# alexmillerdb/two_tower_recommender_model

Hardware: AMD Instinct MI355X
Metric: training pairs/sec at batch 8192 (per GPU) (higher is better)
Workload: dtype fp32; 1 GPU; northstar: 100M items x 50M users, emb_dim 128, towers [128, 64], single-hot uniform ids; global_batch=8192, per_gpu_batch=8192, emb_dim=128, tower_dtype=bf16 (MFMA, fp32 acc), parallelism=single-gpu hipgraph

## Files before the change

two_tower_recommender_model_amd/csrc/tower.hip:

```cpp
#include <vector>

#include "tt_common.h"
#include "dedup.h"
#include "shard.h"

namespace tt {

typedef __attribute__((ext_vector_type(8))) __bf16 bf16x8;
typedef __attribute__((ext_vector_type(4))) float f32x4;
typedef __attribute__((ext_vector_type(4))) __bf16 bf16x4;

constexpr int TR = 32;
constexpr int MAXW = 128;
constexpr int XCH = 128;
constexpr int LSTR = MAXW + 8;
constexpr int FSTR = MAXW + 4;
constexpr int MAXL = 4;

__device__ __forceinline__ int64_t strip_at(int64_t f, int64_t m, int64_t nf) {
  return (((m >> 5) * nf + f) << 5) + (m & 31);
}

struct TowerArgs {
  tt_tower_shape_t s;
  int64_t B;
  const float* pooled;
  int64_t ldp;
  float* gpooled;
  const float* params;
  const __bf16* wb;
  const __bf16* wtb;
  const __bf16* wbf;
  const __bf16* wtbf;
  int64_t woff[2][MAXL];
  int64_t boff[2][MAXL];
  int64_t wcoff[2][MAXL];
  const void* labels;
  int label_dtype;
  float grad_scale;
  float* logits;
  __bf16* xt;
  __bf16* act;
  __bf16* dzt;
  float* dbpart;
  float* loss_part;
  int64_t in_max;
  int64_t Bp;
  int nwg;
  const void* gcol[2];
  const float* gtab[2];
  int64_t gmod[2];
  int gid_dtype;
  float* pooled_out;
  DedupWs dd;
  int dd_on;
  int dd_table[2];
  const int32_t* gpos[2];
  const float* gsrc[2];
  float* gdst[2];
  const int32_t* gpos_out[2];
  int gsrc_bf16;
  float* uw[2];
  float* us[2];
  float ulr, ueps;
  const void* pcol[2];
  const void* mval;
  const int32_t* moff[2];
  const int32_t* ipos;
  const int32_t* ipos_out;
  const __bf16* isrc;
  float* idst;
  int ifeat0[2];
  int iD;
  const char* wimg;
  tt_peer_direct_t xd;
#if TT_EXPERIMENTS
// ... 1063 lines not shown
  for (int q = 1; q < TT_PEER_MAXW; ++q) {
    if (q < x.W && row >= x.first_row[q]) {
      base = reinterpret_cast<char*>(x.row0[q]);
      f0 = x.first_row[q];
    }
  }
  return base + (row - f0) * row_bytes;
}
__device__ __forceinline__ bool px_copy_unit(const tt_peer_direct_t& x, int64_t u, const uint4*& src, uint4*& dst) {
  int64_t pre = 0;
  bool hit = false;
#pragma unroll
  for (int q = 0; q < TT_PEER_MAXW; ++q) {
    const int64_t n = q < x.W ? x.copy_len[q] >> 4 : 0;
    if (!hit && u >= pre && u < pre + n) {
      src = reinterpret_cast<const uint4*>(x.copy_src[q]) + (u - pre);
      dst = reinterpret_cast<uint4*>(x.copy_dst[q]) + (u - pre);
      hit = true;
    }
    pre += n;
  }
  return hit;
}
__device__ __forceinline__ int64_t px_copy_units(const tt_peer_direct_t& x) {
  int64_t n = 0;
#pragma unroll
  for (int q = 0; q < TT_PEER_MAXW; ++q) n += q < x.W ? x.copy_len[q] >> 4 : 0;
  return n;
}

struct RkRaw {
  uint32_t lo, hi;
};
__device__ __forceinline__ RkRaw rk_raw(const void* p, bool wide, int64_t i) {
  RkRaw r;
  if (wide) {
    const uint2 v = reinterpret_cast<const uint2*>(p)[i];
    r.lo = v.x;
    r.hi = v.y;
  } else {
    r.lo = reinterpret_cast<const uint32_t*>(p)[i];
    r.hi = 0u;
  }
  return r;
}
__device__ __forceinline__ int64_t rk_id(RkRaw r, bool wide) {
  return wide ? (int64_t)(((uint64_t)r.hi << 32) | r.lo) : (int64_t)(int32_t)r.lo;
}
__device__ __forceinline__ float rk_label(RkRaw r, int dt) {
  if (dt == TT_I32) return (float)(int32_t)r.lo;
  if (dt == TT_I64) return (float)(int64_t)(((uint64_t)r.hi << 32) | r.lo);
  return __uint_as_float(r.lo);
}
#if TT_EXPERIMENTS
#define RK_STAMP(k) \
  do { if (a.stamps && lane == 0) a.stamps[8192 + ((int64_t)blockIdx.x * 16 + (k)) * 9 + wid] = (int64_t)__builtin_amdgcn_s_memrealtime(); } while (0)
#define RK_STAMP2(k) \
  do { if (a.stamps && lane == 0) a.stamps[8192 + ((int64_t)blockIdx.x * 16 + (k)) * 9 + 4 + wid] = (int64_t)__builtin_amdgcn_s_memrealtime(); } while (0)
#define RK_STAMP_IMG(k) \
  do { if (a.stamps && lane == 0) a.stamps[8192 + ((int64_t)blockIdx.x * 16 + (k)) * 9 + 8] = (int64_t)__builtin_amdgcn_s_memrealtime(); } while (0)
#else
#define RK_STAMP(k) do { } while (0)
#define RK_STAMP2(k) do { } while (0)
#define RK_STAMP_IMG(k) do { } while (0)
#endif

typedef uint32_t t3_u32x4 __attribute__((ext_vector_type(4)));
constexpr int T3_NSEG = 2 * 2 * MAXL;

struct alignas(64) UpdateArgs {
  float* params;
  float* exp_avg;
  float* exp_avg_sq;
  const float* slab;
  const float* adam_pre;
  const float* grads_in;
  int32_t P;
  int S;
  int do_adam;
  int nseg;
  t3_u32x4 seg[T3_NSEG];
  const float* dbpart;
  int nwg;
  __bf16* wb;
  __bf16* wtb;
  __bf16* wbf;
  __bf16* wtbf;
  int skip_plain;
  float lr, beta1, beta2, eps, wd;
  int64_t* step_state;
  float* grads_out;
  int out_copies;
  int64_t out_stride;
  int64_t out_off[16];
  float out_scale;
  int in_srcs;
  int64_t in_stride;
  char* wimg;
  PxWait wt;
#if TT_EXPERIMENTS
  int64_t* stamps;
#endif
};
#if TT_EXPERIMENTS
#define T3_BLOCK ((int)blockDim.x)
#else
// ... 58 lines not shown
    m = m + (1.f - a.beta1) * (g - m);
    const float v = v0 * a.beta2 + (1.f - a.beta2) * g * g;
    const float denom = sqrtf(v) / bc2_sqrt + a.eps;
    p = p + (-step_size) * m / denom;
    a.exp_avg[i] = m;
    a.exp_avg_sq[i] = v;
    a.params[i] = p;
  }
  if (sg.sisw) {
    const int K = sg.sk, N = sg.sn;
    const int64_t n = e / K, k = e - n * K;
    if (!a.skip_plain) {
      a.wb[sg.swc + e] = (__bf16)p;
      a.wtb[sg.swc + k * N + n] = (__bf16)p;
    }
    a.wbf[sg.swc + frag_off((int)n, (int)k, K)] = (__bf16)p;
    a.wtbf[sg.swc + frag_off((int)k, (int)n, N)] = (__bf16)p;
    if (a.wimg)
      *reinterpret_cast<__bf16*>(a.wimg + sg.st_ * RK_IMG_T + sg.sl_ * (RK_W0 * 256) + rk_off((int)n, (int)k)) = (__bf16)p;
  }
}

template <bool UPD, bool IDX, int IN, bool POOL = false>
__device__ __forceinline__ void tower_rows_body(const TowerArgs& a) {
  static_assert(IN == 128 || IN == 64, "row-owned T1: inputs of 128 or 64");
  static_assert(!POOL || (!UPD && !IDX), "pooled input: the plain T1 only");
  constexpr int NI = IN / 32;
  constexpr int MTI = IN / 16;
  __shared__ __attribute__((aligned(16))) char wimg[RK_IMG];
  __shared__ __attribute__((aligned(16))) float xo[2][2][16 * 64];
  __shared__ float bsum[2][RK_W0 + RK_W1];
  __shared__ float lrow[TR];
  __shared__ __attribute__((aligned(16))) float xr[4][16 * IN];
  const int lane = threadIdx.x & 63, wid = __builtin_amdgcn_readfirstlane(threadIdx.x >> 6);
  typedef __attribute__((address_space(3))) void lds_void;
  typedef __attribute__((address_space(1))) void glb_void;
  if (wid == 4) {
    RK_STAMP_IMG(0);
    if (!TDBG(16)) {
#pragma unroll
      for (int k = 0; k < RK_IMG / 1024; ++k)
        __builtin_amdgcn_global_load_lds((glb_void*)(a.wimg + k * 1024 + lane * 16), (lds_void*)(wimg + k * 1024), 16, 0, 0);
    }
    RK_STAMP_IMG(1);
    __builtin_amdgcn_s_waitcnt(0x0F70);
    RK_STAMP_IMG(2);
    __syncthreads();
    RK_STAMP_IMG(3);
    __syncthreads();
    __syncthreads();
    return;
  }
  const int t = wid >> 1, h = wid & 1, q = lane >> 4, n = lane & 15;
  const int tile = xcd_remap((int)blockIdx.x, (int)gridDim.x);
  const int64_t B = a.B, m0 = (int64_t)tile * TR, m = m0 + 16 * h + n;
  const bool live = m < B;
  RK_STAMP(0);
  const bool wide = a.gid_dtype == TT_I64;
  const int64_t mc = live ? m : 0;
  RkRaw id_raw{0u, 0u}, pout_raw{0u, 0u};
  if (IDX) {
    id_raw.lo = (uint32_t)(t ? a.gpos[1] : a.gpos[0])[mc];
    pout_raw.lo = a.gpos_out[0] ? (uint32_t)(t ? a.gpos_out[1] : a.gpos_out[0])[mc] : id_raw.lo;
  } else if (!POOL) {
    id_raw = rk_raw(t ? a.gcol[1] : a.gcol[0], wide, mc);
  }
  int32_t cl = -1;
  if (UPD) cl = a.dd.claim[live ? t * B + m : 0];
  const RkRaw lab_raw = rk_raw(a.labels, a.label_dtype == TT_I64, mc);
  f32x4 b0v[8], b1v[4];
  auto load_biases = [&]() {
    const float* b0p = a.params + a.boff[t][0];
    const float* b1p = a.params + a.boff[t][1];
#pragma unroll
    for (int mt = 0; mt < 8; ++mt) b0v[mt] = *reinterpret_cast<const f32x4*>(b0p + 32 * (mt >> 1) + 8 * q + 4 * (mt & 1));
#pragma unroll
    for (int mt = 0; mt < 4; ++mt) b1v[mt] = *reinterpret_cast<const f32x4*>(b1p + 32 * (mt >> 1) + 8 * q + 4 * (mt & 1));
  };
  load_biases();
  __builtin_amdgcn_sched_barrier(0);
  uint4 cpv = make_uint4(0u, 0u, 0u, 0u);
  uint4* cpd = nullptr;
  int64_t cp_per = 0, cp_end = 0;
  if constexpr (IDX) {
    if (a.xd.W) {
      const int64_t tot = px_copy_units(a.xd);
      cp_per = (tot + gridDim.x - 1) / gridDim.x;
      cp_end = min(tot, ((int64_t)blockIdx.x + 1) * cp_per);
      const int64_t u = (int64_t)blockIdx.x * cp_per + threadIdx.x;
      const uint4* cps;
      if (u < cp_end && px_copy_unit(a.xd, u, cps, cpd)) cpv = *cps;
      else cpd = nullptr;
    }
  }
  int64_t r;
  if (POOL) {
    r = live ? m : -1;
  } else if (IDX) {
    r = live ? (int64_t)(int32_t)id_raw.lo : -1;
  } else {
    const int64_t id = live ? rk_id(id_raw, wide) : 0;
    r = id != 0 ? py_mod64(id, t ? a.gmod[1] : a.gmod[0]) : -1;
  }
  const float* tab = POOL ? a.pooled + a.s.in_col[t] : (t ? a.gtab[1] : a.gtab[0]);
  const int64_t rstride = POOL ? a.ldp : IN;
  float* xw = xr[wid];
  constexpr int CPR = IDX ? IN / 8 : IN / 4;
  constexpr int RPI = 64 / CPR;
  if (IDX) {
    const int rr0 = lane / CPR, pc = lane % CPR;
    const char* src0 = reinterpret_cast<const char*>(t ? a.gsrc[1] : a.gsrc[0]);
#pragma unroll
    for (int i = 0; i < 16 / RPI; ++i) {
      const int row = RPI * i + rr0;
      const int64_t rid = __shfl((long long)r, row, 64);
      const char* src = src0 + (rid >= 0 ? rid : 0) * (IN * 2) + 16 * (pc ^ (row & (CPR - 1)));
      __builtin_amdgcn_global_load_lds((glb_void*)src, (lds_void*)(reinterpret_cast<char*>(xw) + i * 1024), 16, 0, 0);
    }
  } else {
    const int rr0 = lane / CPR, pc = lane % CPR;
#pragma unroll
    for (int i = 0; i < 16 / RPI; ++i) {
      const int row = RPI * i + rr0;
      const int64_t rid = __shfl((long long)r, row, 64);
      const float* src = tab + (rid >= 0 ? rid : 0) * rstride + 4 * (pc ^ row);
      if (!TDBG(32))
        __builtin_amdgcn_global_load_lds((glb_void*)src, (lds_void*)(xw + i * 256), 16, 0, 0);
    }
  }
  __builtin_amdgcn_sched_barrier(0);
  DdPend pend;
  pend.key = DD_EMPTY;
  const int32_t li = (int32_t)(t * B + m);
  if (!UPD && a.dd_on && q == 0 && live) {
    const uint64_t key = r >= 0 ? (((uint64_t)(t ? a.dd_table[1] : a.dd_table[0]) << DD_TABLE_SHIFT) | (uint64_t)r)
                                : DD_EMPTY;
    dd_insert_begin(a.dd, key, li, pend);
  }
  RK_STAMP(1);
  __builtin_amdgcn_s_waitcnt(0x0F70);
  RK_STAMP(2);
  __syncthreads();
  RK_STAMP(3);
  f32x4 xv[8];
  bf16x8 xb[4];
  if (IDX) {
#pragma unroll
    for (int s2 = 0; s2 < NI; ++s2) {
      const bf16x8 v = *reinterpret_cast<const bf16x8*>(reinterpret_cast<const char*>(xw) + n * (IN * 2) +
                                                         16 * ((4 * s2 + q) ^ (n & (CPR - 1))));
      xb[s2] = r >= 0 ? v : (bf16x8)(__bf16)0.f;
    }
  } else {
#pragma unroll
    for (int mt = 0; mt < MTI; ++mt) {
      const int c = 8 * (mt >> 1) + 2 * q + (mt & 1);
      const f32x4 v = *reinterpret_cast<const f32x4*>(xw + n * IN + 4 * (c ^ n));
      xv[mt] = r >= 0 ? v : (f32x4)(0.f);
    }
#pragma unroll
    for (int s2 = 0; s2 < NI; ++s2) xb[s2] = rk_pack(xv[2 * s2], xv[2 * s2 + 1]);
  }
  uint32_t word = 0u;
  float s_old = 0.f;
  if (UPD) {
    if (blockIdx.x == 0 && threadIdx.x == 0) {
      const int32_t nh = a.dd.ctr[0];
      a.dd.ctr[2] = nh;
      a.dd.ctr[0] = 0;
    }
    word = reinterpret_cast<const uint32_t*>(&a.dd.slots[cl >= 0 ? cl : 0].word)[0];
    s_old = (t ? a.us[1] : a.us[0])[r >= 0 ? r : 0];
  }
  __builtin_amdgcn_sched_barrier(0);
  const char* img0 = wimg + t * RK_IMG_T;
  const char* img1 = img0 + RK_W0 * 256;
  f32x4 acc[8];
  if (!TDBG(512)) rk_strip<NI>(xb, a.xt + (int64_t)t * a.in_max * a.Bp + m * a.in_max, q);
  rk_gemm<8, NI, false>(acc, img0, xb, lane);
  RK_STAMP(4);
  bf16x8 hb[4];
#pragma unroll
  for (int s = 0; s < 4; ++s) {
    f32x4 u0, u1;
#pragma unroll
    for (int j = 0; j < 4; ++j) {
      u0[j] = fmaxf(acc[2 * s][j] + b0v[2 * s][j], 0.f);
      u1[j] = fmaxf(acc[2 * s + 1][j] + b0v[2 * s + 1][j], 0.f);
    }
    hb[s] = rk_pack(u0, u1);
  }
  if (!TDBG(256)) rk_strip<4>(hb, a.act + ((int64_t)t * MAXL + 0) * MAXW * a.Bp + m * MAXW, q);
  f32x4 uo[4];
  rk_gemm<4, 4, false>(acc, img1, hb, lane);
#pragma unroll
  for (int mt = 0; mt < 4; ++mt) uo[mt] = acc[mt];
#pragma unroll
  for (int mt = 0; mt < 4; ++mt) {
#pragma unroll
    for (int j = 0; j < 4; ++j) uo[mt][j] = fmaxf(uo[mt][j] + b1v[mt][j], 0.f);
    const int c = 8 * (mt >> 1) + 2 * q + (mt & 1);
    *reinterpret_cast<f32x4*>(&xo[t][h][n * 64 + ((c ^ n) << 2)]) = uo[mt];
  }
  RK_STAMP(5);
  RK_STAMP(6);
  __syncthreads();
  RK_STAMP(7);
  f32x4 vo[4];
#pragma unroll
  for (int mt = 0; mt < 4; ++mt) {
    const int c = 8 * (mt >> 1) + 2 * q + (mt & 1);
    vo[mt] = *reinterpret_cast<const f32x4*>(&xo[t ^ 1][h][n * 64 + ((c ^ n) << 2)]);
  }
  float gs[4];
#pragma unroll
  for (int mt = 0; mt < 4; ++mt) {
    float e = 0.f;
#pragma unroll
    for (int j = 0; j < 4; ++j) e = fmaf(uo[mt][j], vo[mt][j], e);
    gs[mt] = e;
  }
  float c0 = gs[0] + gs[1], c1 = gs[2] + gs[3];
  c0 += __shfl_xor(c0, 16, 64);
  c1 += __shfl_xor(c1, 16, 64);
  c0 += __shfl_xor(c0, 32, 64);
  c1 += __shfl_xor(c1, 32, 64);
  const float d = c0 + c1;
  float lo = 0.f, dl = 0.f;
  if (live) {
    const float x = d, y = rk_label(lab_raw, a.label_dtype);
    const float e = __expf(-fabsf(x));
    const float l1p = e < 1e-4f ? e * (1.f - 0.5f * e) : __logf(1.f + e);
    const float lsig = fminf(x, 0.f) - l1p;
    lo = (1.f - y) * x - lsig;
    const float rc = __builtin_amdgcn_rcpf(1.f + e);
    dl = ((x >= 0.f ? rc : e * rc) - y) * (a.grad_scale / (float)B);
  }
  if (t == 0 && q == 0) lrow[16 * h + n] = lo;
  float z1[16];
  bf16x8 z1b[4];
#pragma unroll
  for (int mt = 0; mt < 4; ++mt)
#pragma unroll
    for (int j = 0; j < 4; ++j) z1[4 * mt + j] = live && uo[mt][j] > 0.f ? dl * vo[mt][j] : 0.f;
#pragma unroll
  for (int s = 0; s < 2; ++s) {
    bf16x8 v;
#pragma unroll
    for (int j = 0; j < 8; ++j) v[j] = (__bf16)z1[8 * s + j];
    z1b[s] = v;
  }
  RK_STAMP(8);
  rk_gemm<8, 2, true>(acc, img1, z1b, lane);
  float z0[32];
  bf16x8 z0b[4];
#pragma unroll
  for (int mt = 0; mt < 8; ++mt)
#pragma unroll
    for (int j = 0; j < 4; ++j)
      z0[4 * mt + j] = live && (float)hb[mt >> 1][4 * (mt & 1) + j] > 0.f ? acc[mt][j] : 0.f;
#pragma unroll
  for (int s = 0; s < 4; ++s) {
    bf16x8 v;
#pragma unroll
    for (int j = 0; j < 8; ++j) v[j] = (__bf16)z0[8 * s + j];
    z0b[s] = v;
  }
  if (!TDBG(512)) rk_strip<2>(z1b, a.dzt + ((int64_t)t * MAXL + 1) * MAXW * a.Bp + m * MAXW, q);
  if (!TDBG(128)) rk_strip<4>(z0b, a.dzt + ((int64_t)t * MAXL + 0) * MAXW * a.Bp + m * MAXW, q);
  RK_STAMP(9);
  rk_gemm<MTI, 4, true>(acc, img0, z0b, lane);
  RK_STAMP(10);
  float* grow;
  bool store_dx;
  if (IDX) {
    const int32_t po = (int32_t)pout_raw.lo;
    store_dx = r >= 0 && po >= 0;
    grow = (t ? a.gdst[1] : a.gdst[0]) + (int64_t)(store_dx ? po : 0) * IN;
    if (a.xd.W) grow = reinterpret_cast<float*>(px_row(a.xd, store_dx ? po : 0, IN * 4));
  } else {
    grow = live ? a.gpooled + m * a.ldp + a.s.in_col[t] : nullptr;
    store_dx = live;
  }
  if (UPD) {
    float e2[2];
#pragma unroll
    for (int hh = 0; hh < 2; ++hh) {
      const float s0 = rw_sq4(acc[0 + hh]), s1 = rw_sq4(acc[2 + hh]);
      float c2;
      if constexpr (IN == 128) {
        const float s2 = rw_sq4(acc[4 + hh]), s3 = rw_sq4(acc[6 + hh]);
        c2 = (s0 + s2) + (s1 + s3);
      } else {
        c2 = s0 + s1;
      }
      c2 += __shfl_xor(c2, 32, 64);
      c2 += __shfl_xor(c2, 16, 64);
      e2[hh] = c2;
    }
    RK_STAMP2(0);
    const float sq = e2[0] + e2[1];
    const float snew = rw_state(s_old, sq, IN);
    const float step = rw_step(snew, a.ulr, a.ueps);
    const uint32_t cnt = word & (uint32_t)DD_CNT_MASK;
    const bool single = r >= 0 && cl >= 0 && cnt == 1u;
    {
      const bool mul = q == 0 && r >= 0 && cl >= 0 && cnt >= 2u && cnt <= (uint32_t)DD_INL;
      const uint64_t bal = __ballot(mul);
      const int seg = tile * 4 + wid;
      if (seg < a.dd.nseg) {
        if (mul) a.dd.multi[(int64_t)seg * DD_SEGW + 1 + __popcll(bal & ((1ull << lane) - 1))] = cl;
        if (lane == 0) a.dd.multi[(int64_t)seg * DD_SEGW] = __popcll(bal);
      }
    }
#pragma unroll
    for (int mt = 0; mt < MTI; ++mt) {
      const int c = 8 * (mt >> 1) + 2 * q + (mt & 1);
      *reinterpret_cast<f32x4*>(xw + n * IN + 4 * (c ^ n)) = rw_apply(xv[mt], acc[mt], step);
    }
    RK_STAMP2(1);
    asm volatile("" ::: "memory");
    {
      const int rr0 = lane / CPR, pc = lane % CPR;
      float* wtab = t ? a.uw[1] : a.uw[0];
#pragma unroll
      for (int i = 0; i < 16 / RPI; ++i) {
        const int row = RPI * i + rr0;
        const int64_t rid = __shfl((long long)r, row, 64);
        const int sg = __shfl((int)single, row, 64);
        const f32x4 w = *reinterpret_cast<const f32x4*>(xw + row * IN + 4 * pc);
        if (sg) *reinterpret_cast<f32x4*>(wtab + rid * IN + 4 * (pc ^ row)) = w;
      }
    }
    RK_STAMP2(2);
    if (single) {
      if (q == 0) {
        (t ? a.us[1] : a.us[0])[r] = snew;
        a.dd.slots[cl].word = DD_EMPTY;
      }
      store_dx = a.pooled_out != nullptr;
    }
  }
  if (store_dx) {
#pragma unroll
    for (int mt = 0; mt < MTI; ++mt)
      *reinterpret_cast<f32x4*>(grow + 32 * (mt >> 1) + 8 * q + 4 * (mt & 1)) = acc[mt];
  }
  RK_STAMP2(3);
  if (t == 0 && q == 0 && live) a.logits[m] = d;
  if (!IDX && !POOL && a.pooled_out && live) {
    float* prow = a.pooled_out + m * a.ldp + a.s.in_col[t];
#pragma unroll
    for (int mt = 0; mt < MTI; ++mt) *reinterpret_cast<f32x4*>(prow + 32 * (mt >> 1) + 8 * q + 4 * (mt & 1)) = xv[mt];
  }
  RK_STAMP(11);
  RK_STAMP(12);
  rk_colsum<32>(z0, n);
  rk_colsum<16>(z1, n);
  auto feat = [&](int k) { return 32 * ((k >> 2) >> 1) + 8 * q + 4 * ((k >> 2) & 1) + (k & 3); };
  if (h == 1) {
    bsum[t][feat(2 * n)] = z0[0];
    bsum[t][feat(2 * n + 1)] = z0[1];
    bsum[t][RK_W0 + feat(n)] = z1[0];
  }
  RK_STAMP(13);
  __syncthreads();
  RK_STAMP(14);
  if (h == 0) {
    float* db0 = a.dbpart + (((int64_t)t * MAXL + 0) * a.nwg + tile) * MAXW;
    float* db1 = a.dbpart + (((int64_t)t * MAXL + 1) * a.nwg + tile) * MAXW;
    db0[feat(2 * n)] = z0[0] + bsum[t][feat(2 * n)];
    db0[feat(2 * n + 1)] = z0[1] + bsum[t][feat(2 * n + 1)];
    db1[feat(n)] = z1[0] + bsum[t][RK_W0 + feat(n)];
    if (t == 0 && lane == 0) {
      float p = 0.f;
      for (int i = 0; i < TR; ++i) p += lrow[i];
      a.loss_part[tile] = p;
    }
  }
  if (!UPD && a.dd_on && q == 0) dd_insert_defer_finish_at(a.dd, pend, li, tile, 16 * wid + n);
  if constexpr (IDX) {
    if (cpd) *cpd = cpv;
    if (a.xd.W) {
      for (int64_t u = (int64_t)blockIdx.x * cp_per + threadIdx.x + 256; u < cp_end; u += 256) {
        const uint4* s2;
        uint4* d2;
        if (px_copy_unit(a.xd, u, s2, d2)) *d2 = *s2;
      }
    }
    if (a.xd.epoch && blockIdx.x == 0 && threadIdx.x == 0)
      __hip_atomic_fetch_add(a.xd.epoch, 1, __ATOMIC_RELAXED, __HIP_MEMORY_SCOPE_AGENT);
  }
  RK_STAMP(15);
}
template <bool UPD, bool IDX = false, int IN = 128, bool POOL = false>
__global__ void __launch_bounds__(RK_THREADS) tower_rows_kernel(TowerArgs a) {
  tower_rows_body<UPD, IDX, IN, POOL>(a);
}


struct WgradTile {
  int32_t t, l, n0, k0;
};


struct WgradArgs {
  const __bf16* xt;
  const __bf16* act;
  const __bf16* dzt;
  float* slab;
  int64_t P;
  int64_t B;
  int64_t in_max;
  int64_t Bp;
  int S;
  int64_t mslice;
  int ntiles;
  int64_t woff[2][MAXL];
  int64_t boff[2][MAXL];
  int32_t K[2][MAXL];
  int32_t width[MAXL];
  int L;
  const float* dbpart;
  int nwg;
  const float* loss_part;
  float* loss;
  int nbias;
  int64_t tiles_off;
  int64_t* step_state;
  float* adam_pre;
// ... 932 lines not shown
  if (rc) return rc;
  hipStream_t st = as_stream(stream);
  char* ws = reinterpret_cast<char*>(workspace);
  if (hipMemsetAsync(ws, 0, L.total, st) != hipSuccess) return fail(TT_EINVAL, "tower: memset failed");
  if (L.lds) return hipStreamSynchronize(st) == hipSuccess ? TT_OK : fail(TT_EINVAL, "tower: init sync failed");
  std::vector<WgradTile> tiles;
  for (int t = 0; t < 2; ++t)
    for (int l = 0; l < shape->L; ++l)
      for (int n0 = 0; n0 < shape->width[l]; n0 += 32)
        for (int k0 = 0; k0 < L.K[t][l]; k0 += 32) tiles.push_back({t, l, n0, k0});
  if (hipMemcpyAsync(ws + L.o_tiles, tiles.data(), tiles.size() * sizeof(WgradTile), hipMemcpyHostToDevice, st) !=
      hipSuccess)
    return fail(TT_EINVAL, "tower: tile upload failed");
  return hipStreamSynchronize(st) == hipSuccess ? TT_OK : fail(TT_EINVAL, "tower: init sync failed");
}

}

namespace tt {
static int insert_args(const tt_insert_role_t& in, int64_t B, const char* what, InsertArgs& ins) {
  const std::string w(what);
  if (!in.next_cols || !in.num_embeddings || !in.dedup_tables || !in.next_dedup_ws)
    return fail(TT_EINVAL, w + ": null pointer");
  if (in.id_dtype != TT_I32 && in.id_dtype != TT_I64) return fail(TT_EINVAL, w + ": ids must be int32/int64");
  if (int rc = check_dedup_ws(in.next_dedup_ws, in.dedup_ws_bytes, in.dedup_max_lookups, 2 * B, what, true)) return rc;
  for (int t = 0; t < 2; ++t) {
    if (!in.next_cols[t] || in.num_embeddings[t] < 1 || in.num_embeddings[t] >= (1ll << DD_TABLE_SHIFT) ||
        in.dedup_tables[t] < 0 || in.dedup_tables[t] >= TT_MAX_TABLES)
      return fail(TT_EINVAL, "tower insert: bad column / table");
    ins.col[t] = in.next_cols[t];
    ins.mod[t] = in.num_embeddings[t];
    ins.tab[t] = in.dedup_tables[t];
  }
  ins.id_dtype = in.id_dtype;
  ins.B = B;
  ins.xcd_wpt = (INS_PT == 1 && B % 2048 == 0) ? (int)(B / 2048) : 0;
  dedup_layout(in.next_dedup_ws, in.dedup_max_lookups, &ins.dd);
  return TT_OK;
}

}

namespace tt {
struct T1Common {
  const float* params;
  const void* labels;
  int label_dtype;
  float grad_scale;
  float* logits;
  void* workspace;
  size_t ws_bytes;
  void* stream;
};

static int launch_t1(const tt_tower_shape_t* shape, int64_t B, TowerArgs& a, const float* pooled, int64_t ldp,
                     float* gpooled, const T1Common& c) {
  const float* params = c.params;
  const void* labels = c.labels;
  const int label_dtype = c.label_dtype;
  const float grad_scale = c.grad_scale;
  float* logits = c.logits;
  void* workspace = c.workspace;
  const size_t ws_bytes = c.ws_bytes;
  void* stream = c.stream;
  TowerLayout L;
  int rc = tower_ws_layout(shape, B, workspace, ws_bytes, &L);
  if (rc) return rc;
  if ((!pooled && !a.gcol[0] && !a.gpos[0] && !a.mval && !a.ipos) || (!gpooled && !a.gpos[0] && !a.ipos) || !params ||
      !labels || !logits)
    return fail(TT_EINVAL, "tower: null pointer");
  if (label_dtype != TT_I32 && label_dtype != TT_I64 && label_dtype != TT_F32)
    return fail(TT_EINVAL, "tower: labels must be int32/int64/float32");
  if (ldp % 4 || (reinterpret_cast<uintptr_t>(pooled) & 15) || (reinterpret_cast<uintptr_t>(gpooled) & 15) ||
      (reinterpret_cast<uintptr_t>(a.pooled_out) & 15))
    return fail(TT_EINVAL, "tower: pooled rows and their gradient must be 16-B aligned");
  for (int t = 0; t < 2; ++t)
    if (shape->in_col[t] + shape->in_dim[t] > ldp) return fail(TT_EINVAL, "tower: input columns exceed the pooled row");
  char* ws = reinterpret_cast<char*>(workspace);
  a.s = *shape;
  a.B = B;
  a.pooled = pooled;
  a.ldp = ldp;
  a.gpooled = gpooled;
  a.params = params;
  a.wb = reinterpret_cast<const __bf16*>(ws + L.o_wb);
  a.wtb = reinterpret_cast<const __bf16*>(ws + L.o_wtb);
  a.wbf = reinterpret_cast<const __bf16*>(ws + L.o_wbf);
  a.wtbf = reinterpret_cast<const __bf16*>(ws + L.o_wtbf);
  for (int t = 0; t < 2; ++t)
    for (int l = 0; l < MAXL; ++l) {
      a.woff[t][l] = L.woff[t][l];
      a.boff[t][l] = L.boff[t][l];
      a.wcoff[t][l] = L.wcoff[t][l];
    }
  a.labels = labels;
  a.label_dtype = label_dtype;
  a.grad_scale = grad_scale;
  a.logits = logits;
  a.xt = reinterpret_cast<__bf16*>(ws + L.o_xt);
  a.act = reinterpret_cast<__bf16*>(ws + L.o_act);
  a.dzt = reinterpret_cast<__bf16*>(ws + L.o_dzt);
  a.dbpart = reinterpret_cast<float*>(ws + L.o_dbpart);
  a.loss_part = reinterpret_cast<float*>(ws + L.o_losspart);
  a.in_max = L.in_max;
  a.Bp = L.Bp;
  a.nwg = L.nwg;
#if TT_EXPERIMENTS
  if (const char* e = getenv("TT_T1_DEBUG")) a.dbg = atoi(e);
  if (a.dbg & 8) a.stamps = reinterpret_cast<int64_t*>(ws + L.o_dbg);
#endif
  const int i0 = shape->in_dim[0], i1 = shape->in_dim[1], w0 = shape->width[0], w1 = shape->width[1];
  const dim3 g(L.nwg), b512(T1_THREADS);
  const bool two = shape->L == 2 && i0 <= 128 && i1 <= 128;
  if ((a.gcol[0] || a.gpos[0]) && !two)
    return fail(TT_EINVAL, "tower: the fused gather needs 2 layers and inputs <= 128 wide");
  if ((shape->flags & TT_TOWER_GENERAL_T1) && !a.ipos)
    return fail(TT_EINVAL, "tower: TT_TOWER_GENERAL_T1 shapes run T1 through tt_tower_fwd_bwd_indexed_multi only");
  if (a.ipos) {
    tower_fwd_bwd_kernel<<<dim3(L.nwg), dim3(256), 0, as_stream(stream)>>>(a);
    return check_launch("tower_fwd_bwd_indexed_multi");
  }
  if (a.mval) {
    if (two && i0 == 128 && i1 == 128 && w0 == 128 && w1 == 64)
      tower_l2_kernel<128, 128, 64, false, false, true><<<g, b512, 0, as_stream(stream)>>>(a);
    else if (two && i0 == 64 && i1 == 64 && w0 == 128 && w1 == 64)
      tower_l2_kernel<64, 128, 64, false, false, true><<<g, b512, 0, as_stream(stream)>>>(a);
    else
      return fail(TT_EINVAL, "tower_fwd_bwd_kjt: shapes in {64, 128} x [128, 64] only");
    return check_launch("tower_fwd_bwd_kjt");
  }
  bool rows_t1 = L.rows && !a.ipos && !a.mval && ((a.gcol[0] && !a.gpos[0]) || (a.gpos[0] && a.gsrc_bf16));
  const bool rows_pool = L.rows && !a.ipos && !a.mval && !a.gcol[0] && !a.gpos[0] && pooled &&
                         !(reinterpret_cast<uintptr_t>(pooled) & 15);
  bool rows_pool_ok = true;
#if TT_EXPERIMENTS
  if (getenv("TT_T1_CLASSIC")) rows_t1 = false;
#endif
  if (rows_t1) {
    a.wimg = ws + L.o_wimg;
    if (a.gpos[0])
      i0 == 64 ? tower_rows_kernel<false, true, 64><<<g, dim3(RK_THREADS), 0, as_stream(stream)>>>(a)
               : tower_rows_kernel<false, true, 128><<<g, dim3(RK_THREADS), 0, as_stream(stream)>>>(a);
    else if (a.uw[0])
      i0 == 64 ? tower_rows_kernel<true, false, 64><<<g, dim3(RK_THREADS), 0, as_stream(stream)>>>(a)
               : tower_rows_kernel<true, false, 128><<<g, dim3(RK_THREADS), 0, as_stream(stream)>>>(a);
    else
      i0 == 64 ? tower_rows_kernel<false, false, 64><<<g, dim3(RK_THREADS), 0, as_stream(stream)>>>(a)
               : tower_rows_kernel<false, false, 128><<<g, dim3(RK_THREADS), 0, as_stream(stream)>>>(a);
    return check_launch(a.uw[0] ? "tower_rows_gather_update" : "tower_rows_gather");
  }
#if TT_EXPERIMENTS
  if (getenv("TT_T1_CLASSIC")) rows_pool_ok = false;
#endif
  if (rows_pool && rows_pool_ok) {
    a.wimg = ws + L.o_wimg;
    i0 == 64 ? tower_rows_kernel<false, false, 64, true><<<g, dim3(RK_THREADS), 0, as_stream(stream)>>>(a)
             : tower_rows_kernel<false, false, 128, true><<<g, dim3(RK_THREADS), 0, as_stream(stream)>>>(a);
    return check_launch("tower_rows_pooled");
  }
  if (a.uw[0]) {
    if (two && i0 == 128 && i1 == 128 && w0 == 128 && w1 == 64)
      tower_l2_kernel<128, 128, 64, false, true><<<g, b512, 0, as_stream(stream)>>>(a);
    else if (two && i0 == 64 && i1 == 64 && w0 == 128 && w1 == 64)
      tower_l2_kernel<64, 128, 64, false, true><<<g, b512, 0, as_stream(stream)>>>(a);
    else
      return fail(TT_EINVAL, "tower_gather_update: shapes in {64, 128} x [128, 64] only");
    return check_launch("tower_fwd_bwd_gather_update");
  }
  if (two && i0 == 128 && i1 == 128 && w0 == 128 && w1 == 64 && a.gsrc_bf16)
    tower_l2_kernel<128, 128, 64, true><<<g, b512, 0, as_stream(stream)>>>(a);
  else if (two && a.gsrc_bf16)
    tower_l2_kernel<0, 0, 0, true><<<g, b512, 0, as_stream(stream)>>>(a);
  else if (two && i0 == 128 && i1 == 128 && w0 == 128 && w1 == 64)
    tower_l2_kernel<128, 128, 64><<<g, b512, 0, as_stream(stream)>>>(a);
  else if (two && i0 == 64 && i1 == 64 && w0 == 128 && w1 == 64)
    tower_l2_kernel<64, 128, 64><<<g, b512, 0, as_stream(stream)>>>(a);
  else if (two)
    tower_l2_kernel<0, 0, 0><<<g, b512, 0, as_stream(stream)>>>(a);
  else
    tower_fwd_bwd_kernel<<<dim3(L.nwg), dim3(256), 0, as_stream(stream)>>>(a);
  return check_launch("tower_fwd_bwd");
}

static int wgrad_args(const tt_tower_shape_t* shape, int64_t B, void* workspace, size_t ws_bytes,
                      const tt_wgrad_role_t& w, WgradArgs& a, int64_t* wgs, TowerLayout& L) {
  int rc = tower_ws_layout(shape, B, workspace, ws_bytes, &L);
  if (rc) return rc;
  char* ws = reinterpret_cast<char*>(workspace);
  a.xt = reinterpret_cast<const __bf16*>(ws + L.o_xt);
  a.act = reinterpret_cast<const __bf16*>(ws + L.o_act);
  a.dzt = reinterpret_cast<const __bf16*>(ws + L.o_dzt);
  a.slab = reinterpret_cast<float*>(ws + L.o_slab);
  a.P = L.P;
  a.B = B;
  a.in_max = L.in_max;
  a.Bp = L.Bp;
  a.S = L.S;
  a.mslice = L.mslice;
  a.ntiles = L.ntiles;
  for (int t = 0; t < 2; ++t)
    for (int l = 0; l < MAXL; ++l) {
      a.woff[t][l] = L.woff[t][l];
      a.boff[t][l] = L.boff[t][l];
      a.K[t][l] = L.K[t][l];
    }
  int nbias = 0;
  for (int l = 0; l < shape->L; ++l) {
    a.width[l] = shape->width[l];
// ... 653 lines not shown
```

Measured before the change: 291.3 million pairs/s.

## Pack per-tower rows-kernel args into cache-line front block with pinned scalar loads

```diff
diff --git a/two_tower_recommender_model_amd/csrc/tower.hip b/two_tower_recommender_model_amd/csrc/tower.hip
--- a/two_tower_recommender_model_amd/csrc/tower.hip
+++ b/two_tower_recommender_model_amd/csrc/tower.hip
@@ -21,7 +21,55 @@
   return (((m >> 5) * nf + f) << 5) + (m & 31);
 }
 
-struct TowerArgs {
+struct alignas(64) RkTower {
+  const void* idcol;
+  const void* tab;
+  int64_t gmod;
+  const float* b0;
+  const float* b1;
+  const int32_t* claim;
+  const int32_t* pos_out;
+  int64_t rstride;
+  __bf16* xt;
+  __bf16* act0;
+  float* us;
+  __bf16* dzt0;
+  __bf16* dzt1;
+  float* grow;
+  float* prow;
+  int64_t pad1_;
+  float* uw;
+  float* db0;
+  float* db1;
+  int64_t pad2_[5];
+};
+struct alignas(64) RkCommon {
+  int64_t B;
+  const void* labels;
+  int32_t label_dtype;
+  int32_t gid_dtype;
+  float grad_scale;
+  int32_t in_max;
+  DSlot* slots;
+  int32_t* ctr;
+  float ulr, ueps;
+  int32_t nwg;
+  float fB;
+  int64_t ldp;
+  int32_t* multi;
+  float* logits;
+  float* loss_part;
+  int32_t nseg;
+  int32_t pad1_[7];
+};
+struct RkFront {
+  RkCommon c;
+  RkTower tw[2];
+};
+static_assert(sizeof(RkTower) == 192 && sizeof(RkCommon) == 128, "whole 64-B lines");
+
+struct alignas(64) TowerArgs {
+  RkFront rk;
   tt_tower_shape_t s;
   int64_t B;
   const float* pooled;
@@ -1191,6 +1239,16 @@
   if (dt == TT_I64) return (float)(int64_t)(((uint64_t)r.hi << 32) | r.lo);
   return __uint_as_float(r.lo);
 }
+template <int N, typename T>
+__device__ __forceinline__ void rk_pin(T (&p)[N]) {
+  static_assert(N == 2 || N == 4 || N == 8, "2, 4 or 8 values");
+  if constexpr (N == 8)
+    asm volatile("" : "+v"(p[0]), "+v"(p[1]), "+v"(p[2]), "+v"(p[3]), "+v"(p[4]), "+v"(p[5]), "+v"(p[6]), "+v"(p[7]));
+  else if constexpr (N == 4)
+    asm volatile("" : "+v"(p[0]), "+v"(p[1]), "+v"(p[2]), "+v"(p[3]));
+  else
+    asm volatile("" : "+v"(p[0]), "+v"(p[1]));
+}
 #if TT_EXPERIMENTS
 #define RK_STAMP(k) \
   do { if (a.stamps && lane == 0) a.stamps[8192 + ((int64_t)blockIdx.x * 16 + (k)) * 9 + wid] = (int64_t)__builtin_amdgcn_s_memrealtime(); } while (0)
@@ -1355,26 +1413,42 @@
     return;
   }
   const int t = wid >> 1, h = wid & 1, q = lane >> 4, n = lane & 15;
-  const int tile = xcd_remap((int)blockIdx.x, (int)gridDim.x);
-  const int64_t B = a.B, m0 = (int64_t)tile * TR, m = m0 + 16 * h + n;
+  const RkCommon& C = a.rk.c;
+  const RkTower& T = a.rk.tw[t];
+  const int64_t B = C.B;
+  const void* const labels = C.labels;
+  const int label_dtype = C.label_dtype, gid_dtype = C.gid_dtype;
+  const void* const idcol = T.idcol;
+  const void* const tab0 = T.tab;
+  const int64_t gmod = T.gmod;
+  const float* const b0p = T.b0;
+  const float* const b1p = T.b1;
+  const int32_t* const claim = T.claim;
+  const int32_t* const pos_out = T.pos_out;
+  const int64_t pstride = T.rstride;
+  const int nwg = C.nwg;
+  if (UPD) asm volatile("" ::"s"(nwg), "s"(B), "s"(labels), "s"(label_dtype), "s"(gid_dtype), "s"(idcol), "s"(tab0), "s"(gmod), "s"(b0p), "s"(b1p), "s"(claim));
+  else if (IDX) asm volatile("" ::"s"(nwg), "s"(B), "s"(labels), "s"(label_dtype), "s"(idcol), "s"(tab0), "s"(b0p), "s"(b1p), "s"(pos_out));
+  else if (POOL) asm volatile("" ::"s"(nwg), "s"(B), "s"(labels), "s"(label_dtype), "s"(tab0), "s"(b0p), "s"(b1p), "s"(pstride));
+  else asm volatile("" ::"s"(nwg), "s"(B), "s"(labels), "s"(label_dtype), "s"(gid_dtype), "s"(idcol), "s"(tab0), "s"(gmod), "s"(b0p), "s"(b1p));
+  const int tile = xcd_remap((int)blockIdx.x, nwg);
+  const int64_t m0 = (int64_t)tile * TR, m = m0 + 16 * h + n;
   const bool live = m < B;
   RK_STAMP(0);
-  const bool wide = a.gid_dtype == TT_I64;
+  const bool wide = gid_dtype == TT_I64;
   const int64_t mc = live ? m : 0;
   RkRaw id_raw{0u, 0u}, pout_raw{0u, 0u};
   if (IDX) {
-    id_raw.lo = (uint32_t)(t ? a.gpos[1] : a.gpos[0])[mc];
-    pout_raw.lo = a.gpos_out[0] ? (uint32_t)(t ? a.gpos_out[1] : a.gpos_out[0])[mc] : id_raw.lo;
+    id_raw.lo = (uint32_t) reinterpret_cast<const int32_t*>(idcol)[mc];
+    pout_raw.lo = pos_out ? (uint32_t)pos_out[mc] : id_raw.lo;
   } else if (!POOL) {
-    id_raw = rk_raw(t ? a.gcol[1] : a.gcol[0], wide, mc);
+    id_raw = rk_raw(idcol, wide, mc);
   }
   int32_t cl = -1;
-  if (UPD) cl = a.dd.claim[live ? t * B + m : 0];
-  const RkRaw lab_raw = rk_raw(a.labels, a.label_dtype == TT_I64, mc);
+  if (UPD) cl = claim[mc];
+  const RkRaw lab_raw = rk_raw(labels, label_dtype == TT_I64, mc);
   f32x4 b0v[8], b1v[4];
   auto load_biases = [&]() {
-    const float* b0p = a.params + a.boff[t][0];
-    const float* b1p = a.params + a.boff[t][1];
 #pragma unroll
     for (int mt = 0; mt < 8; ++mt) b0v[mt] = *reinterpret_cast<const f32x4*>(b0p + 32 * (mt >> 1) + 8 * q + 4 * (mt & 1));
 #pragma unroll
@@ -1403,33 +1477,50 @@
     r = live ? (int64_t)(int32_t)id_raw.lo : -1;
   } else {
     const int64_t id = live ? rk_id(id_raw, wide) : 0;
-    r = id != 0 ? py_mod64(id, t ? a.gmod[1] : a.gmod[0]) : -1;
-  }
-  const float* tab = POOL ? a.pooled + a.s.in_col[t] : (t ? a.gtab[1] : a.gtab[0]);
-  const int64_t rstride = POOL ? a.ldp : IN;
+    r = id != 0 ? py_mod64(id, gmod) : -1;
+  }
+  const float* tab = reinterpret_cast<const float*>(tab0);
+  const int64_t rstride = POOL ? pstride : IN;
+  RK_STAMP2(4);
+  __builtin_amdgcn_sched_barrier(0);
   float* xw = xr[wid];
   constexpr int CPR = IDX ? IN / 8 : IN / 4;
   constexpr int RPI = 64 / CPR;
+  constexpr int NDMA = 16 / RPI;
   if (IDX) {
     const int rr0 = lane / CPR, pc = lane % CPR;
-    const char* src0 = reinterpret_cast<const char*>(t ? a.gsrc[1] : a.gsrc[0]);
-#pragma unroll
-    for (int i = 0; i < 16 / RPI; ++i) {
+    const char* src0 = reinterpret_cast<const char*>(tab0);
+    const char* src[NDMA];
+    int64_t rid[NDMA];
+#pragma unroll
+    for (int i = 0; i < NDMA; ++i) rid[i] = __shfl((long long)r, RPI * i + rr0, 64);
+    rk_pin<NDMA>(rid);
+#pragma unroll
+    for (int i = 0; i < NDMA; ++i) {
       const int row = RPI * i + rr0;
-      const int64_t rid = __shfl((long long)r, row, 64);
-      const char* src = src0 + (rid >= 0 ? rid : 0) * (IN * 2) + 16 * (pc ^ (row & (CPR - 1)));
-      __builtin_amdgcn_global_load_lds((glb_void*)src, (lds_void*)(reinterpret_cast<char*>(xw) + i * 1024), 16, 0, 0);
-    }
+      src[i] = src0 + (rid[i] >= 0 ? rid[i] : 0) * (IN * 2) + 16 * (pc ^ (row & (CPR - 1)));
+    }
+    rk_pin<NDMA>(src);
+#pragma unroll
+    for (int i = 0; i < NDMA; ++i)
+      __builtin_amdgcn_global_load_lds((glb_void*)src[i], (lds_void*)(reinterpret_cast<char*>(xw) + i * 1024), 16, 0, 0);
   } else {
     const int rr0 = lane / CPR, pc = lane % CPR;
-#pragma unroll
-    for (int i = 0; i < 16 / RPI; ++i) {
+    const float* src[NDMA];
+    int64_t rid[NDMA];
+#pragma unroll
+    for (int i = 0; i < NDMA; ++i) rid[i] = __shfl((long long)r, RPI * i + rr0, 64);
+    rk_pin<NDMA>(rid);
+#pragma unroll
+    for (int i = 0; i < NDMA; ++i) {
       const int row = RPI * i + rr0;
-      const int64_t rid = __shfl((long long)r, row, 64);
-      const float* src = tab + (rid >= 0 ? rid : 0) * rstride + 4 * (pc ^ row);
+      src[i] = tab + (rid[i] >= 0 ? rid[i] : 0) * rstride + 4 * (pc ^ row);
+    }
+    rk_pin<NDMA>(src);
+#pragma unroll
+    for (int i = 0; i < NDMA; ++i)
       if (!TDBG(32))
-        __builtin_amdgcn_global_load_lds((glb_void*)src, (lds_void*)(xw + i * 256), 16, 0, 0);
-    }
+        __builtin_amdgcn_global_load_lds((glb_void*)src[i], (lds_void*)(xw + i * 256), 16, 0, 0);
   }
   __builtin_amdgcn_sched_barrier(0);
   DdPend pend;
@@ -1441,7 +1532,16 @@
     dd_insert_begin(a.dd, key, li, pend);
   }
   RK_STAMP(1);
+  const int in_max = C.in_max;
+  const float grad_scale = C.grad_scale, fB = C.fB;
+  DSlot* const slots = C.slots;
+  __bf16* const xt_t = T.xt;
+  __bf16* const act_t = T.act0;
+  const float* const us_t = T.us;
+  __builtin_amdgcn_sched_barrier(0);
   __builtin_amdgcn_s_waitcnt(0x0F70);
+  if (UPD) asm volatile("" ::"s"(in_max), "s"(grad_scale), "s"(fB), "s"(slots), "s"(xt_t), "s"(act_t), "s"(us_t));
+  else asm volatile("" ::"s"(in_max), "s"(grad_scale), "s"(fB), "s"(xt_t), "s"(act_t));
   RK_STAMP(2);
   __syncthreads();
   RK_STAMP(3);
@@ -1468,18 +1568,19 @@
   float s_old = 0.f;
   if (UPD) {
     if (blockIdx.x == 0 && threadIdx.x == 0) {
-      const int32_t nh = a.dd.ctr[0];
-      a.dd.ctr[2] = nh;
-      a.dd.ctr[0] = 0;
-    }
-    word = reinterpret_cast<const uint32_t*>(&a.dd.slots[cl >= 0 ? cl : 0].word)[0];
-    s_old = (t ? a.us[1] : a.us[0])[r >= 0 ? r : 0];
+      int32_t* const ctr = C.ctr;
+      const int32_t nh = ctr[0];
+      ctr[2] = nh;
+      ctr[0] = 0;
+    }
+    word = reinterpret_cast<const uint32_t*>(&slots[cl >= 0 ? cl : 0].word)[0];
+    s_old = us_t[r >= 0 ? r : 0];
   }
   __builtin_amdgcn_sched_barrier(0);
   const char* img0 = wimg + t * RK_IMG_T;
   const char* img1 = img0 + RK_W0 * 256;
   f32x4 acc[8];
-  if (!TDBG(512)) rk_strip<NI>(xb, a.xt + (int64_t)t * a.in_max * a.Bp + m * a.in_max, q);
+  if (!TDBG(512)) rk_strip<NI>(xb, xt_t + m * in_max, q);
   rk_gemm<8, NI, false>(acc, img0, xb, lane);
   RK_STAMP(4);
   bf16x8 hb[4];
@@ -1493,7 +1594,7 @@
     }
     hb[s] = rk_pack(u0, u1);
   }
-  if (!TDBG(256)) rk_strip<4>(hb, a.act + ((int64_t)t * MAXL + 0) * MAXW * a.Bp + m * MAXW, q);
+  if (!TDBG(256)) rk_strip<4>(hb, act_t + m * MAXW, q);
   f32x4 uo[4];
   rk_gemm<4, 4, false>(acc, img1, hb, lane);
 #pragma unroll
@@ -1531,15 +1632,16 @@
   const float d = c0 + c1;
   float lo = 0.f, dl = 0.f;
   if (live) {
-    const float x = d, y = rk_label(lab_raw, a.label_dtype);
+    const float x = d, y = rk_label(lab_raw, label_dtype);
     const float e = __expf(-fabsf(x));
     const float l1p = e < 1e-4f ? e * (1.f - 0.5f * e) : __logf(1.f + e);
     const float lsig = fminf(x, 0.f) - l1p;
     lo = (1.f - y) * x - lsig;
     const float rc = __builtin_amdgcn_rcpf(1.f + e);
-    dl = ((x >= 0.f ? rc : e * rc) - y) * (a.grad_scale / (float)B);
-  }
-  if (t == 0 && q == 0) lrow[16 * h + n] = lo;
+    dl = ((x >= 0.f ? rc : e * rc) - y) * (grad_scale / fB);
+  }
+  const int hv = (int)(threadIdx.x >> 6) & 1;
+  if (t == 0 && q == 0) lrow[16 * hv + n] = lo;
   float z1[16];
   bf16x8 z1b[4];
 #pragma unroll
@@ -1554,7 +1656,15 @@
     z1b[s] = v;
   }
   RK_STAMP(8);
+  __bf16* const dzt0_t = T.dzt0;
+  __bf16* const dzt1_t = T.dzt1;
+  float* const uw_t = T.uw;
+  const float ulr = C.ulr, ueps = C.ueps;
+  int32_t* const multi = C.multi;
+  const int nseg = C.nseg;
   rk_gemm<8, 2, true>(acc, img1, z1b, lane);
+  if (UPD) asm volatile("" ::"s"(dzt0_t), "s"(dzt1_t), "s"(uw_t), "s"(ulr), "s"(ueps), "s"(multi), "s"(nseg));
+  else asm volatile("" ::"s"(dzt0_t), "s"(dzt1_t));
   float z0[32];
   bf16x8 z0b[4];
 #pragma unroll
@@ -1569,20 +1679,36 @@
     for (int j = 0; j < 8; ++j) v[j] = (__bf16)z0[8 * s + j];
     z0b[s] = v;
   }
-  if (!TDBG(512)) rk_strip<2>(z1b, a.dzt + ((int64_t)t * MAXL + 1) * MAXW * a.Bp + m * MAXW, q);
-  if (!TDBG(128)) rk_strip<4>(z0b, a.dzt + ((int64_t)t * MAXL + 0) * MAXW * a.Bp + m * MAXW, q);
+  if (!TDBG(512)) rk_strip<2>(z1b, dzt1_t + m * MAXW, q);
+  if (!TDBG(128)) rk_strip<4>(z0b, dzt0_t + m * MAXW, q);
   RK_STAMP(9);
+  float* grow_t = nullptr;
+  float* prow_t = nullptr;
+  int64_t ldp = 0;
+  float* db0_t = nullptr;
+  float* db1_t = nullptr;
+  float* logits = nullptr;
+  float* loss_part = nullptr;
+  if constexpr (!UPD) {
+    grow_t = T.grow;
+    prow_t = T.prow;
+    ldp = C.ldp;
+    db0_t = T.db0;
+    db1_t = T.db1;
+    logits = C.logits;
+    loss_part = C.loss_part;
+  }
   rk_gemm<MTI, 4, true>(acc, img0, z0b, lane);
+  if constexpr (!UPD) asm volatile("" ::"s"(grow_t), "s"(prow_t), "s"(ldp), "s"(db0_t), "s"(db1_t), "s"(logits), "s"(loss_part));
   RK_STAMP(10);
-  float* grow;
+  float* grow = nullptr;
   bool store_dx;
   if (IDX) {
     const int32_t po = (int32_t)pout_raw.lo;
     store_dx = r >= 0 && po >= 0;
-    grow = (t ? a.gdst[1] : a.gdst[0]) + (int64_t)(store_dx ? po : 0) * IN;
+    grow = grow_t + (int64_t)(store_dx ? po : 0) * IN;
     if (a.xd.W) grow = reinterpret_cast<float*>(px_row(a.xd, store_dx ? po : 0, IN * 4));
   } else {
-    grow = live ? a.gpooled + m * a.ldp + a.s.in_col[t] : nullptr;
     store_dx = live;
   }
   if (UPD) {
@@ -1604,16 +1730,16 @@
     RK_STAMP2(0);
     const float sq = e2[0] + e2[1];
     const float snew = rw_state(s_old, sq, IN);
-    const float step = rw_step(snew, a.ulr, a.ueps);
+    const float step = rw_step(snew, ulr, ueps);
     const uint32_t cnt = word & (uint32_t)DD_CNT_MASK;
     const bool single = r >= 0 && cl >= 0 && cnt == 1u;
     {
       const bool mul = q == 0 && r >= 0 && cl >= 0 && cnt >= 2u && cnt <= (uint32_t)DD_INL;
       const uint64_t bal = __ballot(mul);
       const int seg = tile * 4 + wid;
-      if (seg < a.dd.nseg) {
-        if (mul) a.dd.multi[(int64_t)seg * DD_SEGW + 1 + __popcll(bal & ((1ull << lane) - 1))] = cl;
-        if (lane == 0) a.dd.multi[(int64_t)seg * DD_SEGW] = __popcll(bal);
+      if (seg < nseg) {
+        if (mul) multi[(int64_t)seg * DD_SEGW + 1 + __popcll(bal & ((1ull << lane) - 1))] = cl;
+        if (lane == 0) multi[(int64_t)seg * DD_SEGW] = __popcll(bal);
       }
     }
 #pragma unroll
@@ -1625,34 +1751,49 @@
     asm volatile("" ::: "memory");
     {
       const int rr0 = lane / CPR, pc = lane % CPR;
-      float* wtab = t ? a.uw[1] : a.uw[0];
-#pragma unroll
-      for (int i = 0; i < 16 / RPI; ++i) {
+      float* wtab = uw_t;
+      const int64_t rsend = single ? r : -1;
+      int64_t rid[NDMA];
+      f32x4 w[NDMA];
+      grow_t = T.grow;
+      prow_t = T.prow;
+      ldp = C.ldp;
+      db0_t = T.db0;
+      db1_t = T.db1;
+      logits = C.logits;
+      loss_part = C.loss_part;
+#pragma unroll
+      for (int i = 0; i < NDMA; ++i) rid[i] = __shfl((long long)rsend, RPI * i + rr0, 64);
+#pragma unroll
+      for (int i = 0; i < NDMA; ++i) w[i] = *reinterpret_cast<const f32x4*>(xw + (RPI * i + rr0) * IN + 4 * pc);
+      rk_pin<NDMA>(rid);
+      rk_pin<NDMA>(w);
+      asm volatile("" ::"s"(grow_t), "s"(prow_t), "s"(ldp), "s"(db0_t), "s"(db1_t), "s"(logits), "s"(loss_part));
+#pragma unroll
+      for (int i = 0; i < NDMA; ++i) {
         const int row = RPI * i + rr0;
-        const int64_t rid = __shfl((long long)r, row, 64);
-        const int sg = __shfl((int)single, row, 64);
-        const f32x4 w = *reinterpret_cast<const f32x4*>(xw + row * IN + 4 * pc);
-        if (sg) *reinterpret_cast<f32x4*>(wtab + rid * IN + 4 * (pc ^ row)) = w;
+        if (__builtin_expect(rid[i] >= 0, 1)) *reinterpret_cast<f32x4*>(wtab + rid[i] * IN + 4 * (pc ^ row)) = w[i];
       }
     }
     RK_STAMP2(2);
     if (single) {
       if (q == 0) {
-        (t ? a.us[1] : a.us[0])[r] = snew;
-        a.dd.slots[cl].word = DD_EMPTY;
-      }
-      store_dx = a.pooled_out != nullptr;
-    }
-  }
+        const_cast<float*>(us_t)[r] = snew;
+        slots[cl].word = DD_EMPTY;
+      }
+      store_dx = prow_t != nullptr;
+    }
+  }
+  if (!IDX) grow = grow_t + m * ldp;
   if (store_dx) {
 #pragma unroll
     for (int mt = 0; mt < MTI; ++mt)
       *reinterpret_cast<f32x4*>(grow + 32 * (mt >> 1) + 8 * q + 4 * (mt & 1)) = acc[mt];
   }
   RK_STAMP2(3);
-  if (t == 0 && q == 0 && live) a.logits[m] = d;
-  if (!IDX && !POOL && a.pooled_out && live) {
-    float* prow = a.pooled_out + m * a.ldp + a.s.in_col[t];
+  if (t == 0 && q == 0 && live) logits[m] = d;
+  if (!IDX && !POOL && prow_t && live) {
+    float* prow = prow_t + m * ldp;
 #pragma unroll
     for (int mt = 0; mt < MTI; ++mt) *reinterpret_cast<f32x4*>(prow + 32 * (mt >> 1) + 8 * q + 4 * (mt & 1)) = xv[mt];
   }
@@ -1661,7 +1802,7 @@
   rk_colsum<32>(z0, n);
   rk_colsum<16>(z1, n);
   auto feat = [&](int k) { return 32 * ((k >> 2) >> 1) + 8 * q + 4 * ((k >> 2) & 1) + (k & 3); };
-  if (h == 1) {
+  if (hv == 1) {
     bsum[t][feat(2 * n)] = z0[0];
     bsum[t][feat(2 * n + 1)] = z0[1];
     bsum[t][RK_W0 + feat(n)] = z1[0];
@@ -1669,16 +1810,16 @@
   RK_STAMP(13);
   __syncthreads();
   RK_STAMP(14);
-  if (h == 0) {
-    float* db0 = a.dbpart + (((int64_t)t * MAXL + 0) * a.nwg + tile) * MAXW;
-    float* db1 = a.dbpart + (((int64_t)t * MAXL + 1) * a.nwg + tile) * MAXW;
+  if (hv == 0) {
+    float* db0 = db0_t + (int64_t)tile * MAXW;
+    float* db1 = db1_t + (int64_t)tile * MAXW;
     db0[feat(2 * n)] = z0[0] + bsum[t][feat(2 * n)];
     db0[feat(2 * n + 1)] = z0[1] + bsum[t][feat(2 * n + 1)];
     db1[feat(n)] = z1[0] + bsum[t][RK_W0 + feat(n)];
     if (t == 0 && lane == 0) {
       float p = 0.f;
       for (int i = 0; i < TR; ++i) p += lrow[i];
-      a.loss_part[tile] = p;
+      loss_part[tile] = p;
     }
   }
   if (!UPD && a.dd_on && q == 0) dd_insert_defer_finish_at(a.dd, pend, li, tile, 16 * wid + n);
@@ -2717,6 +2858,49 @@
   size_t ws_bytes;
   void* stream;
 };
+
+static void rk_front(TowerArgs& a, bool pool) {
+  RkCommon& c = a.rk.c;
+  c.B = a.B;
+  c.labels = a.labels;
+  c.label_dtype = a.label_dtype;
+  c.gid_dtype = a.gid_dtype;
+  c.grad_scale = a.grad_scale;
+  c.in_max = (int32_t)a.in_max;
+  c.slots = a.dd.slots;
+  c.ctr = a.dd.ctr;
+  c.ulr = a.ulr;
+  c.nwg = a.nwg;
+  c.fB = (float)a.B;
+  c.ueps = a.ueps;
+  c.ldp = a.ldp;
+  c.multi = a.dd.multi;
+  c.logits = a.logits;
+  c.loss_part = a.loss_part;
+  c.nseg = a.dd.nseg;
+  const bool idx = a.gpos[0] != nullptr;
+  for (int t = 0; t < 2; ++t) {
+    RkTower& w = a.rk.tw[t];
+    w.idcol = idx ? static_cast<const void*>(a.gpos[t]) : a.gcol[t];
+    w.tab = idx ? static_cast<const void*>(a.gsrc[t]) : pool ? static_cast<const void*>(a.pooled + a.s.in_col[t]) : a.gtab[t];
+    w.gmod = a.gmod[t];
+    w.b0 = a.params + a.boff[t][0];
+    w.b1 = a.params + a.boff[t][1];
+    w.claim = a.uw[0] ? a.dd.claim + (int64_t)t * a.B : nullptr;
+    w.pos_out = a.gpos_out[0] ? a.gpos_out[t] : nullptr;
+    w.rstride = a.ldp;
+    w.xt = a.xt + (int64_t)t * a.in_max * a.Bp;
+    w.act0 = a.act + ((int64_t)t * MAXL + 0) * MAXW * a.Bp;
+    w.dzt0 = a.dzt + ((int64_t)t * MAXL + 0) * MAXW * a.Bp;
+    w.dzt1 = a.dzt + ((int64_t)t * MAXL + 1) * MAXW * a.Bp;
+    w.us = a.us[t];
+    w.uw = a.uw[t];
+    w.grow = idx ? a.gdst[t] : a.gpooled + a.s.in_col[t];
+    w.prow = a.pooled_out ? a.pooled_out + a.s.in_col[t] : nullptr;
+    w.db0 = a.dbpart + ((int64_t)t * MAXL + 0) * a.nwg * MAXW;
+    w.db1 = a.dbpart + ((int64_t)t * MAXL + 1) * a.nwg * MAXW;
+  }
+}
 
 static int launch_t1(const tt_tower_shape_t* shape, int64_t B, TowerArgs& a, const float* pooled, int64_t ldp,
                      float* gpooled, const T1Common& c) {
@@ -2803,6 +2987,7 @@
 #endif
   if (rows_t1) {
     a.wimg = ws + L.o_wimg;
+    rk_front(a, false);
     if (a.gpos[0])
       i0 == 64 ? tower_rows_kernel<false, true, 64><<<g, dim3(RK_THREADS), 0, as_stream(stream)>>>(a)
                : tower_rows_kernel<false, true, 128><<<g, dim3(RK_THREADS), 0, as_stream(stream)>>>(a);
@@ -2819,6 +3004,7 @@
 #endif
   if (rows_pool && rows_pool_ok) {
     a.wimg = ws + L.o_wimg;
+    rk_front(a, true);
     i0 == 64 ? tower_rows_kernel<false, false, 64, true><<<g, dim3(RK_THREADS), 0, as_stream(stream)>>>(a)
              : tower_rows_kernel<false, false, 128, true><<<g, dim3(RK_THREADS), 0, as_stream(stream)>>>(a);
     return check_launch("tower_rows_pooled");
```

After: 298.3 million pairs/s, median of 6. 2.4% higher.
